# juhyeonkim95/Mitsuba3DopplerToF

Measured on AMD Instinct MI355X. Metric: Mpaths/s (whole node), Doppler Cornell 512x512 64spp, higher is better.
Workload: dtype f32

## Files before the change

mitsuba3dopplertof_amd/__init__.py:

```python
import ctypes as C
import os

import numpy as np

__all__ = ["load_file", "load_string", "load_dict", "Scene", "Integrator", "Sampler", "DtofError", "render",
           "render_multi_pass", "to_tof_image", "lib_path", "ETimeSampling", "velocity_map_variants", "MOMENT_PLANES"]

_HERE = os.path.dirname(os.path.abspath(__file__))
_LIB = None


class DtofError(RuntimeError):
    pass


class ETimeSampling:
    UNIFORM, STRATIFIED, ANTITHETIC, ANTITHETIC_MIRROR, PERIODIC, REGULAR = 0, 1, 2, 3, 4, 5


class _Stats(C.Structure):
    _fields_ = [("n_paths", C.c_uint64), ("n_bounces", C.c_uint64), ("n_shadow_rays", C.c_uint64),
                ("ms_total", C.c_double), ("ms_generate", C.c_double), ("ms_trace", C.c_double),
                ("ms_shade", C.c_double), ("ms_shadow", C.c_double), ("ms_splat", C.c_double),
                ("n_launches_trace", C.c_uint32), ("n_launches_shade", C.c_uint32), ("n_launches_shadow", C.c_uint32),
                ("n_batches", C.c_uint32), ("n_launches_first", C.c_uint32), ("ms_first", C.c_double),
                ("n_inline_iterations", C.c_uint32), ("n_bounces_inline", C.c_uint64), ("n_fused_splat_launches", C.c_uint32),
                ("n_plan_facts_launches", C.c_uint32)]

    def as_dict(self):
        return {k: getattr(self, k) for k, _ in self._fields_}


class _Info(C.Structure):
    _fields_ = [("film_width", C.c_int32), ("film_height", C.c_int32), ("crop_x", C.c_int32), ("crop_y", C.c_int32),
                ("crop_width", C.c_int32), ("crop_height", C.c_int32), ("sample_count", C.c_uint32),
                ("n_shapes", C.c_uint32), ("n_groups", C.c_uint32), ("n_objects", C.c_uint32), ("n_emitters", C.c_uint32),
                ("n_triangles", C.c_uint32), ("n_bvh_nodes", C.c_uint32), ("scene_blob_bytes", C.c_uint32),
                ("time", C.c_float), ("w_g", C.c_float), ("g_1", C.c_float), ("g_0", C.c_float), ("w_s", C.c_float),
                ("phase_offset", C.c_float), ("hetero_frequency", C.c_float), ("antithetic_shift", C.c_float),
                ("wave_type", C.c_int32), ("low_frequency_component_only", C.c_int32), ("time_sampling", C.c_int32),
                ("stratify_each_interval", C.c_int32), ("path_correlation_depth", C.c_uint32), ("max_depth", C.c_uint32),
                ("rr_depth", C.c_uint32), ("base_seed", C.c_uint32), ("time_correlate_number", C.c_int32),
                ("path_correlate_number", C.c_int32), ("bvh_stack_depth", C.c_uint32),
                ("filter_radius", C.c_float), ("filter_halo", C.c_int32), ("has_alpha", C.c_int32)]


_FLAT_SHAPE_FIELDS = 1 << 18 | 0xf << 19 | 0x7 << 23


def lib_path():
    return os.environ.get("DTOF_LIB") or os.path.join(_HERE, "libdtof.so")


def _lib():
    global _LIB
    if _LIB is not None:
        return _LIB
    path = lib_path()
    try:
        import torch
    except ImportError:
        pass
    if not os.path.exists(path):
        raise ImportError("%s is missing -- build it with `make -C %s/csrc` (or __graft_entry__.build()); "
                          "there is no CPU fallback" % (path, _HERE))
    L = C.CDLL(path)
    cpp = C.POINTER(C.c_char_p)
    vp = C.c_void_p
    L.dtof_version.restype = C.c_char_p
    L.dtof_last_error.restype = C.c_char_p
# ... 193 lines not shown

    def info(self):
        i = _Info()
        _check(_lib().dtof_scene_get_info(self._h, C.byref(i)))
        return {k: getattr(i, k) for k, _ in i._fields_}

    @property
    def size(self):
        i = self.info()
        return i["crop_width"], i["crop_height"]

    def export(self, kind):
        n = C.c_size_t(0)
        _check(_lib().dtof_scene_export(self._h, kind, None, 0, C.byref(n)))
        out = np.zeros(n.value, np.float32)
        _check(_lib().dtof_scene_export(self._h, kind, out.ctypes.data, out.size, C.byref(n)))
        return out

    @property
    def plan_facts_launches(self):
        return int(_lib().dtof_scene_plan_facts_launches(self._h))

    @property
    def last_plan_mask(self):
        return int(_lib().dtof_scene_last_plan_facts(self._h))

    @property
    def last_plan_facts(self):
        return self.last_plan_mask & ~_FLAT_SHAPE_FIELDS

    @property
    def last_plan_shape(self):
        m = self.last_plan_mask
        return ((m >> 19) & 0xf, (m >> 23) & 0x7) if m & (1 << 18) else None

    def set_integrator(self, props):
        _check(_lib().dtof_scene_set_integrator(self._h, *_plugin_args(props)))

    def set_sampler(self, props):
        _check(_lib().dtof_scene_set_sampler(self._h, *_plugin_args(props)))

    def render(self, seed=0, spp=0, offsets=None, sensor=0, variants=None, film="float32"):
        if offsets is not None and variants is not None:
            raise DtofError("pass either offsets or variants, not both")
        if _film64(film):
            if sensor != 0:
                raise DtofError("Scene::render(): sensor index %d is out of bounds!" % sensor)
            if offsets is not None:
# ... 442 lines not shown
```

mitsuba3dopplertof_amd/csrc/dtof_kernels.h:

```cpp
#pragma once
#include <stdint.h>
#include <hip/hip_runtime.h>
#include "dtof_math.h"

namespace dtof {

constexpr uint32_t kChunkBlocks = 8;
constexpr uint32_t kMaxInline = 4;
constexpr int kMaxOffsets = 4;

struct RenderParams {
    float s2c[16];
    float cam_to_world[12];
    float near_clip, far_clip, shutter_open, shutter_open_time;
    int32_t orthographic;
    float aperture_radius, focus_distance;
    int32_t crop_x, crop_y, crop_w, crop_h;
    float scale_x, scale_y, offset_x, offset_y;
    int32_t filter; float filter_radius, inv_radius;
    float gauss_coeff[10];
    float filter_b, filter_c;
    uint32_t base_seed, seed, seed_value;
    uint32_t spp, spp_log2;
    uint32_t tcn, pcn;
// ... 99 lines not shown
static_assert(ShadeLds::resident(171, 8, false, true, 12).bytes() == 103088 && ShadeLds::resident(171, 8, false, true, 12).park_off() == 3072, "resident stage, four films");
static_assert(ShadeLds::classic(214, true, true, 5).bytes() == 10080 && ShadeLds::classic(214, true, true, 5).without_stack() == 9568, "classic one-wall launch");

enum : uint32_t {
    kFactSinglePass     = 1u << 0,
    kFactDopplerCorr    = 1u << 1,
    kFactNoLaneOutput   = 1u << 2,
    kFactIdentityQueue  = 1u << 3,
    kFactNoRoulette     = 1u << 4,
    kFactCorrelated     = 1u << 5,
    kFactWholePath      = 1u << 6,
    kFactOneBlock       = 1u << 7,
    kFactOneEmitter     = 1u << 8,
    kFactWavePixel      = 1u << 9,
    kFactFlat           = 1u << 10,
    kFactOneWall        = 1u << 11,
    kFactFusedSplat     = 1u << 12,
    kFactStratifiedPairs = 1u << 13,
    kFactPow2Strata     = 1u << 14,
    kFactSineLowPass    = 1u << 15,
    kFactEmitterSampled = 1u << 16,
    kFactIdShift24      = 1u << 17,
    kFactFlatShape      = 1u << 18,
};
constexpr uint32_t kFlatShapeCountShift = 19, kFlatShapeWallShift = 23, kFlatShapeMax = 8;
constexpr uint32_t kFlatShapeFields = kFactFlatShape | 0xfu << kFlatShapeCountShift | 0x7u << kFlatShapeWallShift;
constexpr uint32_t flat_shape_fact(uint32_t n_objects, uint32_t wall) {
    return n_objects >= 1 && n_objects <= kFlatShapeMax && wall < n_objects ? kFactFlatShape | n_objects << kFlatShapeCountShift | wall << kFlatShapeWallShift : 0u;
}
constexpr uint32_t flat_shape_count(uint32_t facts) { return (facts & kFactFlatShape) ? (facts >> kFlatShapeCountShift) & 0xfu : 0u; }
constexpr uint32_t flat_shape_wall(uint32_t facts) { return (facts >> kFlatShapeWallShift) & 0x7u; }
constexpr bool facts_hold(uint32_t launch, uint32_t kernel) {
    return (launch & kernel & ~kFlatShapeFields) == (kernel & ~kFlatShapeFields) && (!(kernel & kFactFlatShape) || (launch & kFlatShapeFields) == (kernel & kFlatShapeFields));
}
constexpr uint32_t kFactsFlatTable = kFactOneWall | kFlatShapeFields;
static_assert(flat_shape_fact(5, 2) == 0x12c0000u && flat_shape_count(flat_shape_fact(5, 2)) == 5 && flat_shape_wall(flat_shape_fact(5, 2)) == 2 && flat_shape_fact(9, 2) == 0 && flat_shape_fact(5, 5) == 0, "shape fields");
constexpr uint32_t kFactsSampling = kFactStratifiedPairs | kFactPow2Strata | kFactSineLowPass | kFactEmitterSampled | kFactIdShift24;
constexpr bool facts_lane_shifts(uint32_t facts) { return (facts & kFactWavePixel) != 0 && (facts & kFactsSampling) != 0; }
#ifndef DTOF_HEADLINE_FACTS
#define DTOF_HEADLINE_FACTS 0xfff
#endif
constexpr uint32_t kHeadlineFacts = DTOF_HEADLINE_FACTS;
#ifndef DTOF_HEADLINE_FUSED
#define DTOF_HEADLINE_FUSED 1
#endif
constexpr uint32_t kHeadlineFusedFacts = DTOF_HEADLINE_FUSED ? (kHeadlineFacts | kFactFusedSplat) : 0u;
#ifndef DTOF_HEADLINE_C2
#define DTOF_HEADLINE_C2 0x3e000
#endif
constexpr uint32_t kHeadlineC2Facts = (DTOF_HEADLINE_C2) != 0 && kHeadlineFusedFacts != 0 ? (kHeadlineFusedFacts | (DTOF_HEADLINE_C2)) : 0u;
static_assert(((DTOF_HEADLINE_C2) & ~kFactsSampling) == 0, "DTOF_HEADLINE_C2 names route facts only (bits 13 and up)");
#ifndef DTOF_HEADLINE_SHAPE_COUNT
#define DTOF_HEADLINE_SHAPE_COUNT 5
#endif
#ifndef DTOF_HEADLINE_SHAPE_WALL
#define DTOF_HEADLINE_SHAPE_WALL 2
#endif
constexpr uint32_t kHeadlineShapeFacts = (DTOF_HEADLINE_SHAPE_COUNT) != 0 && (kHeadlineC2Facts & kFactOneWall) != 0 ? (kHeadlineC2Facts | flat_shape_fact(DTOF_HEADLINE_SHAPE_COUNT, DTOF_HEADLINE_SHAPE_WALL)) : 0u;
static_assert((DTOF_HEADLINE_SHAPE_COUNT) == 0 || (kHeadlineC2Facts & kFactOneWall) == 0 || (kHeadlineShapeFacts & kFactFlatShape) != 0, "a shape has 1 .. 8 objects and the wall among them");
#ifndef DTOF_FLAT_SHAPE_ANY
#define DTOF_FLAT_SHAPE_ANY 1
#endif
#ifndef DTOF_FLAT_SHAPE_CLOSEST
#define DTOF_FLAT_SHAPE_CLOSEST 1
#endif
#ifndef DTOF_WALL_FRAMES
#define DTOF_WALL_FRAMES 1
#endif
#ifndef DTOF_RESIDENT_FACTS
#define DTOF_RESIDENT_FACTS 0x37f
#endif
constexpr uint32_t kResidentFacts = DTOF_RESIDENT_FACTS;

struct ShadeLaunch { bool staged; int mode; uint32_t waves, grid, lds, lds_flat; hipStream_t stream; ShadeArgs args; uint32_t facts; };
uint32_t launch_shade_plain(bool area, bool k4, const ShadeLaunch &L);
void launch_shade_mesh(bool area, bool k4, const ShadeLaunch &L);
void launch_shade_spec1(bool k4, const ShadeLaunch &L);
void launch_shade_spec2(bool k4, const ShadeLaunch &L);
uint32_t launch_shade_resident0(bool area, bool k4, const ShadeLaunch &L);
void launch_shade_resident1(bool k4, const ShadeLaunch &L);
void launch_shade_resident2(bool k4, const ShadeLaunch &L);

// ... 70 lines not shown
```

mitsuba3dopplertof_amd/csrc/dtof_math.h:

```cpp
#pragma once
#include <hip/hip_runtime.h>
#include <stdint.h>
#include <math.h>

#define DTOF_HD __host__ __device__ __forceinline__

namespace dtof {

constexpr float kPi = 3.14159265358979323846f;
constexpr float kInvPi = 0.31830988618379067154f;
constexpr float kRayEps = 1500.f * 5.9604644775390625e-8f;
constexpr float kShadowEps = kRayEps * 10.f;
constexpr float kLargest = 3.40282346638528859812e+38f;

struct V3 { float x, y, z; };

DTOF_HD uint32_t f2u(float f) {
#if defined(__HIP_DEVICE_COMPILE__)
    return __float_as_uint(f);
#else
    uint32_t u; __builtin_memcpy(&u, &f, 4); return u;
#endif
}
DTOF_HD float u2f(uint32_t u) {
// ... 372 lines not shown
        sum += 0x9e3779b9u;
        v0 += ((v1 << 4) + 0xa341316cu) ^ (v1 + sum) ^ ((v1 >> 5) + 0xc8013ea4u);
        v1 += ((v0 << 4) + 0xad90777du) ^ (v0 + sum) ^ ((v0 >> 5) + 0x7e95761eu);
    }
    o0 = v0; o1 = v1;
}
constexpr uint64_t kPcgMult = 0x5851f42d4c957f2dULL;
DTOF_HD uint32_t pcg_next_u32(uint64_t &state, uint64_t inc) {
    uint64_t old = state;
    state = old * kPcgMult + inc;
    uint32_t xs = (uint32_t) (((old >> 18) ^ old) >> 27), rot = (uint32_t) (old >> 59);
    return (xs >> rot) | (xs << ((~rot + 1u) & 31));
}
DTOF_HD float pcg_next_f32(uint64_t &state, uint64_t inc) {
    return u2f((pcg_next_u32(state, inc) >> 9) | 0x3f800000u) - 1.f;
}
DTOF_HD float pcg_output_f32(uint64_t old) {
    uint32_t xs = (uint32_t) (((old >> 18) ^ old) >> 27), rot = (uint32_t) (old >> 59);
    return u2f((((xs >> rot) | (xs << ((~rot + 1u) & 31))) >> 9) | 0x3f800000u) - 1.f;
}
constexpr uint64_t pcg_pow(int n) { uint64_t r = 1; for (int i = 0; i < n; ++i) r *= kPcgMult; return r; }
constexpr uint64_t kPcgMult6 = pcg_pow(6), kPcgGeom6 = 1 + pcg_pow(1) + pcg_pow(2) + pcg_pow(3) + pcg_pow(4) + pcg_pow(5);
DTOF_HD uint64_t pcg_jump6(uint64_t state, uint64_t inc) { return state * kPcgMult6 + inc * kPcgGeom6; }
DTOF_HD void pcg_seed(uint32_t initstate, uint32_t initseq, uint64_t &state, uint64_t &inc) {
    state = 0; inc = ((uint64_t) initseq << 1) | 1u;
    pcg_next_u32(state, inc);
    state += (uint64_t) initstate;
    pcg_next_u32(state, inc);
}
DTOF_HD uint32_t permute_kensler(uint32_t index, uint32_t n, uint32_t seed, FastDiv dn) {
    if (n <= 1) return 0;
    uint32_t w = n - 1;
    w |= w >> 1; w |= w >> 2; w |= w >> 4; w |= w >> 8; w |= w >> 16;
    do {
        uint32_t tmp = index;
        tmp ^= seed;            tmp *= 0xe170893du;
        tmp ^= seed >> 16;      tmp ^= (tmp & w) >> 4;
        tmp ^= seed >> 8;       tmp *= 0x0929eb3fu;
        tmp ^= seed >> 23;      tmp ^= (tmp & w) >> 1;
        tmp *= 1 | seed >> 27;  tmp *= 0x6935fa69u;
        tmp ^= (tmp & w) >> 11; tmp *= 0x74dcb303u;
        tmp ^= (tmp & w) >> 2;  tmp *= 0x9e501cc3u;
        tmp ^= (tmp & w) >> 2;  tmp *= 0xc860a3dfu;
        tmp &= w;               tmp ^= tmp >> 5;
        index = tmp;
    } while (index >= n);
// ... 20 lines not shown
```

mitsuba3dopplertof_amd/csrc/dtof_render.hip:

```cpp
#include "../../include/dtof.h"
#include "dtof_kernels.h"
#include "dtof_reconstruct.h"
#include "dtof_film64.h"
#include "dtof_moments.h"
#include "dtof_flat_query.h"
#include "dtof_scene.h"
#include "dtof_math.h"
#include <atomic>
#include <dlfcn.h>
#include <cstdio>
#include <cstring>
#include <cstdlib>
#include <cmath>
#include <string>
#include <memory>
#include <vector>

using namespace dtof;

namespace {

thread_local std::string g_last_error;

struct HipError : std::runtime_error { using std::runtime_error::runtime_error; };
// ... 390 lines not shown
    }
    uint32_t launch_facts(const RenderParams &r, const LaunchSpan &l, uint32_t depth0, bool first, bool identity_queue, bool dump) const {
        if (!plan_facts || !first) return 0u;
        const uint32_t depth_end = depth0 + l.span;
        uint32_t f = 0;
        if (r.n_passes == 1 && r.pass == 0) f |= kFactSinglePass;
        if (r.integrator == 0 && r.sampler_kind == SAMPLER_CORRELATED) f |= kFactDopplerCorr;
        if (!dump && !r.want_valid) f |= kFactNoLaneOutput;
        if (identity_queue) f |= kFactIdentityQueue;
        if (r.rr_depth > depth_end) f |= kFactNoRoulette;
        if (depth_end < r.path_correlation_depth) f |= kFactCorrelated;
        if (!l.next_runs && l.terminal) f |= kFactWholePath;
        if (l.chunk_blocks == 1) f |= kFactOneBlock;
        if (n_emitters == 1) f |= kFactOneEmitter;
        if (r.flat_objects != 0) f |= kFactFlat;
        if (one_wall) f |= kFactOneWall | flat_shape;
        if ((f & kFactDopplerCorr) && r.time_sampling == TIME_STRATIFIED && r.stratify != 0 && r.tcn == 2 && r.pcn == 2 && r.shutter_open_time > 0.f && r.spp > 1) f |= kFactStratifiedPairs;
        if (r.n_stratum >= 2 && (r.n_stratum & (r.n_stratum - 1u)) == 0) f |= kFactPow2Strata;
        if (r.low_pass != 0 && r.wave_type == WAVE_SIN) f |= kFactSineLowPass;
        if (depth_end < r.max_depth) f |= kFactEmitterSampled;
        if (id_shift == 24) f |= kFactIdShift24;
        if (l.splat_here) f |= kFactFusedSplat;
        if (identity_queue && r.stripe_rows == 0 && r.spp_log2 != 0xffffffffu && r.spp_log2 >= 6 && (r.lane_base & 63u) == 0 && (r.n_lanes & 63u) == 0) f |= kFactWavePixel;
        return f;
    }
};

void plan_lanes(FramePlan &p, const dtof_scene *sc, const RenderRequest &rq) {
    const HostSensor &se = sc->host.sensor;
    uint32_t spp = rq.spp ? rq.spp : sc->pp.sample_count;
    if (spp == 0) throw std::runtime_error("sample count must be positive");
    const uint32_t sample_count = spp;
    uint32_t per_pass = sc->pp.samples_per_pass == 0xffffffffu || sc->pp.samples_per_pass == 0 ? spp : std::min(sc->pp.samples_per_pass, spp);
    if (spp % per_pass != 0) throw std::runtime_error("sample_count (" + std::to_string(spp) + ") must be a multiple of spp_per_pass (" + std::to_string(per_pass) + ").");
    const uint64_t wavefront = (uint64_t) se.crop_w * se.crop_h * per_pass, limit = 0xffffffffull;
    if (wavefront > limit) {
        per_pass /= (uint32_t) ((wavefront + limit - 1) / limit);
        if (per_pass == 0 || spp % per_pass != 0) throw std::runtime_error("sample_count should be a multiple of samples_per_wavefront!");
    }
    p.n_passes = spp / per_pass; spp = per_pass;
    const uint64_t total_lanes = (uint64_t) se.crop_w * se.crop_h * spp;
    if (sc->pp.time_sampling != TIME_UNIFORM && sc->pp.stratify_each_interval && sample_count < (uint32_t) sc->pp.time_correlate_number)
        throw std::runtime_error("sample count must be at least time_correlate_number when per-interval stratification is on");
    if (sc->pp.integrator == 0 && sc->pp.sampler_kind == SAMPLER_CORRELATED && sc->pp.time_sampling == TIME_ANTITHETIC_MIRROR && sc->pp.time_correlate_number != 2)
        throw std::runtime_error("antithetic_mirror time sampling needs time_correlate_number == 2");
    p.rp = make_params(sc, rq.seed, spp, rq.offsets, rq.n_offsets, sample_count, rq.variants, rq.n_variants);
// ... 1279 lines not shown
```

mitsuba3dopplertof_amd/csrc/dtof_shade.h:

```cpp
#pragma once
#include "dtof_device.h"
#include <atomic>
#include <initializer_list>
#include <type_traits>

namespace dtof {


DTOF_D uint32_t wave_append(bool pred, uint32_t &running) {
    const uint64_t mask = __ballot(pred);
    const uint32_t slot = running + (uint32_t) __popcll(mask & ((1ull << __lane_id()) - 1ull));
    running += (uint32_t) __popcll(mask);
    return slot;
}

struct BsdfOut { V3 val, weight, wo; float pdf, bs_pdf, bs_eta; bool bs_delta, bs_null; };
template <int SPEC>
DTOF_D void bsdf_eval_pdf_sample(const SceneView &sv, const DShape *sh, Surface &si, V3 wo, bool active_em, float sample_1, float s2x, float s2y, BsdfOut &out, bool want_sample = true) {
    const bool masked = SPEC && (sh->flags & SF_MASK);
    bool null_pick = false; float opacity = 1.f;
    if (masked) { opacity = mask_opacity_at(sv, sh, si.u, si.v); null_pick = !(sample_1 < opacity); sample_1 = sample_1 / opacity; }
    const bool blend = SPEC == 2 && (sh->flags & SF_BLEND);
    float blend_w = 0.f; bool pick_1 = false;
    if (blend) {
        blend_w = sh->tex_blend ? texture_eval_1(sv, sh->tex_blend << 4, si.u, si.v) : sh->blend_weight;
        blend_w = fmin_(fmax_(blend_w, 0.f), 1.f);
        pick_1 = sample_1 <= blend_w;
    }
    const DShape *side_sh = (SPEC == 2 && (sh->flags & SF_TWOSIDED2) && si.wi.z < 0.f) ? &sv.shapes[sh->blend_other] : sh;
    const V3 wi_plain = si.wi, wo_plain = wo;
    V3 bsdf_val = mk(0, 0, 0), bsdf_weight = mk(0, 0, 0), bs_wo = mk(0, 0, 0);
    float bsdf_pdf = 0.f, bs_pdf = 0.f, bs_eta = 0.f; bool bs_delta = false, bs_null = false;
    V3 val_0 = mk(0, 0, 0), keep_weight = mk(0, 0, 0), keep_wo = mk(0, 0, 0); float pdf_0 = 0.f, keep_pdf = 0.f, keep_eta = 0.f; bool keep_delta = false, keep_null = false;
    for (int pass = 0; pass < (SPEC == 2 && blend ? 2 : 1); ++pass) {
        const DShape *bsh = pass ? &sv.shapes[sh->blend_other] : side_sh;
        const float s1 = !blend ? sample_1 : (pass ? sample_1 / blend_w : (sample_1 - blend_w) / (1.f - blend_w));
        si.wi = wi_plain; wo = wo_plain;
        bool twosided = bsh->flags & SF_TWOSIDED;
        const bool nmap = SPEC && (bsh->flags & (SF_NORMALMAP | SF_BUMPMAP));
        LocalFrame nf; V3 wo_flipped = wo; bool nm_back = false;
        if (nmap) {
// ... 152 lines not shown
            }
            if (want_sample && wiz > 0.f) {
                float prob_specular = f_i * w, prob_diffuse = (1.f - f_i) * (1.f - w);
                prob_specular = prob_specular / (prob_specular + prob_diffuse);
                prob_diffuse = 1.f - prob_specular;
                bs_eta = 1.f;
                if (s1 < prob_specular) {
                    bs_wo = mk(-si.wi.x, -si.wi.y, wiz);
                    bs_pdf = prob_specular; bs_delta = true;
                    const float value = f_i / bs_pdf;
                    bsdf_weight = mk(value * hm.spec_refl[0], value * hm.spec_refl[1], value * hm.spec_refl[2]);
                } else {
                    bs_wo = cosine_hemisphere(s2x, s2y);
                    bs_pdf = prob_diffuse * (kInvPi * bs_wo.z);
                    float f_o; fresnel_dielectric(bs_wo.z, bsh->diel_eta, f_o, t1, t2, t3);
                    const float k = bsh->inv_eta_2 * (1.f - f_i) * (1.f - f_o) / prob_diffuse;
                    bsdf_weight = mk(diff.x * k, diff.y * k, diff.z * k);
                }
                if (twosided) bs_wo.z = mulsign(bs_wo.z, si.wi.z);
            }
        } else {
            if (wiz > 0.f && woz > 0.f) { bsdf_val = mk(refl.x * kInvPi * woz, refl.y * kInvPi * woz, refl.z * kInvPi * woz); bsdf_pdf = kInvPi * woz; }
            if (want_sample && wiz > 0.f) {
                bs_wo = cosine_hemisphere(s2x, s2y);
                bs_pdf = kInvPi * bs_wo.z;
                bs_eta = 1.f;
                if (bs_pdf > 0.f) bsdf_weight = refl;
                if (twosided) bs_wo.z = mulsign(bs_wo.z, si.wi.z);
            }
        }
        if (nmap) {
            if (!(wo_flipped.z * wo.z > 0.f)) { bsdf_val = mk(0, 0, 0); bsdf_pdf = 0.f; }
            if (bsdf_weight.x != 0.f || bsdf_weight.y != 0.f || bsdf_weight.z != 0.f) {
                const V3 pw = frame_to_world(nf, bs_wo);
                if (!(bs_wo.z * pw.z > 0.f)) bsdf_weight = mk(0, 0, 0);
                bs_wo = pw;
            }
            if (nm_back) bs_wo.z = -bs_wo.z;
        }
        if (blend) {
            if ((pass == 1) == pick_1) { keep_weight = bsdf_weight; keep_wo = bs_wo; keep_pdf = bs_pdf; keep_eta = bs_eta; keep_delta = bs_delta; keep_null = bs_null; }
            if (pass == 0) { val_0 = bsdf_val; pdf_0 = bsdf_pdf; }
            else {
                const float w0 = 1.f - blend_w;
                bsdf_val = mk(val_0.x * w0 + bsdf_val.x * blend_w, val_0.y * w0 + bsdf_val.y * blend_w, val_0.z * w0 + bsdf_val.z * blend_w);
                bsdf_pdf = pdf_0 * w0 + bsdf_pdf * blend_w;
// ... 62 lines not shown
    }
}
template <bool AREA, bool MESH, int SPEC, bool ONE_EMITTER = false>
void launch_emitter_eval_level(const uint8_t *scene, int mode, uint32_t index, float pmf, const float *in, float *out, uint32_t n, hipStream_t s) {
    if (n) hipLaunchKernelGGL((k_emitter_eval<AREA, MESH, SPEC, ONE_EMITTER>), dim3(nblk(n)), dim3(kBlock), 0, s, scene, mode, index, pmf, in, out, n);
}

template <bool LDS, int MODE, bool AREA, int KMAX, bool MESH, int SPEC, int RESW = 0, bool RH16 = false, uint32_t FACTS = 0>
#ifndef DTOF_MESH_WAVES
#define DTOF_MESH_WAVES 3
#endif
#ifndef DTOF_K4_RES_LDS
#define DTOF_K4_RES_LDS 1
#endif
__global__ __launch_bounds__(RESW ? RESW * 64 : kShadeBlock, RESW ? RESW / 4 : (MODE == 2 && !MESH && !SPEC && KMAX == 1) ? 4 : (MODE != 0 && MESH) ? ((SPEC && KMAX > 1) ? 2 : DTOF_MESH_WAVES) : 1) void k_shade(ShadeArgs args_by_value) {
    constexpr bool FUSED = MODE != 0, FIRST = MODE == 2;
    static_assert(FACTS == 0 || MODE == 2, "plan facts describe a first-bounce launch");
    constexpr bool F_SINGLE_PASS = (FACTS & kFactSinglePass) != 0, F_DOPPLER_CORR = (FACTS & kFactDopplerCorr) != 0, F_NO_LANE_OUT = (FACTS & kFactNoLaneOutput) != 0;
    constexpr bool F_IDENTITY = (FACTS & kFactIdentityQueue) != 0, F_NO_RR = (FACTS & kFactNoRoulette) != 0, F_CORRELATED = (FACTS & kFactCorrelated) != 0;
    constexpr bool F_WHOLE_PATH = (FACTS & kFactWholePath) != 0, F_ONE_BLOCK = (FACTS & kFactOneBlock) != 0, F_ONE_EMITTER = (FACTS & kFactOneEmitter) != 0;
    constexpr bool F_WAVE_PIXEL = (FACTS & kFactWavePixel) != 0;
    constexpr bool F_FLAT = (FACTS & kFactFlat) != 0, F_ONE_WALL = (FACTS & kFactOneWall) != 0, F_FUSED_SPLAT = (FACTS & kFactFusedSplat) != 0;
    constexpr bool F_EMITTER_SAMPLED = (FACTS & kFactEmitterSampled) != 0, F_ID24 = (FACTS & kFactIdShift24) != 0, F_SHIFTS = facts_lane_shifts(FACTS);
    constexpr bool F_FRAMES = F_ONE_WALL && DTOF_WALL_FRAMES;
    static_assert(!F_FLAT || (!MESH && SPEC == 0 && RESW == 0), "trace_flat serves the staged rectangle-only diffuse kernels");
    static_assert(!F_ONE_WALL || F_FLAT, "the one wall is an object of the flat table");
    static_assert(!F_FUSED_SPLAT || KMAX == 1, "the fused splat is the one-film kernels'");
    static_assert(!F_WAVE_PIXEL || F_IDENTITY, "whole waves of one pixel are provable for an identity queue only");
    static_assert(!F_ONE_BLOCK || RESW == 0, "blocks per segment belong to the classic launch");
    constexpr bool RES_LDS = RESW != 0 && KMAX > 1 && DTOF_K4_RES_LDS;
    constexpr bool S16 = RESW != 0 && KMAX > 1;
    static_assert(!RES_LDS || 3 * KMAX == (int) kParkWords + 1, "the film-state columns hold all but the last float of the K results");
    constexpr bool PARK_ST = DTOF_PARK && RESW == 16 && KMAX == 1;
    constexpr bool PARK = DTOF_PARK && RESW == 16 && (KMAX == 1 || RES_LDS);
    constexpr uint32_t kRngAt = RES_LDS ? kParkWords : 0u;
    constexpr int KREG = RES_LDS ? 1 : KMAX;
    constexpr uint32_t kStackStride = RESW ? RESW * 64 : kShadeBlock;
    static_assert(RESW == 0 || (MODE == 2 && !LDS && MESH), "the resident stage exists for the unstaged fused first-bounce kernel with mesh code");
    static_assert(!RH16 || RESW != 0, "half-float LDS planes belong to the resident stage");
    extern __shared__ uint4 lds[];
    __shared__ uint32_t s_inline_all[(RESW ? RESW : 1) * 2 * kMaxInline];
    typedef const char __attribute__((address_space(4))) *KernargBytes;
    const KernargBytes kernarg = (KernargBytes) __builtin_amdgcn_kernarg_segment_ptr();
    const ShadeArgs &A0 = *(const ShadeArgs *) kernarg;
    const uint32_t lane_id = RESW ? threadIdx.x & 63u : threadIdx.x, wave_id = RESW ? threadIdx.x >> 6 : 0u;
    uint32_t *const s_inline = s_inline_all + wave_id * 2 * kMaxInline;
// ... 96 lines not shown
    if constexpr (RES_LDS) res_clear();
    const float4 zero4 = make_float4(0.f, 0.f, 0.f, 0.f);
    uint32_t hid = 0xffffffffu; float4 ra = make_float4(0.f, 0.f, 0.f, 0.f), rb = make_float4(0.f, 0.f, 1.f, 0.f), st = ra; uint4 hh = make_uint4(0u, 0u, 0u, 0u); Rng main = { 0ull, 1ull }, path = { 0ull, 1ull };
    float4 stb_reg = make_float4(0.f, 0.f, 0.f, 1.f); float2 stc_reg = make_float2(1.f, 1.f);
    uint32_t *const parku = (uint32_t *) park;
    auto park_store = [&]() {
        parku[kRngAt * kStackStride] = (uint32_t) main.state; parku[(kRngAt + 1) * kStackStride] = (uint32_t) (main.state >> 32); parku[(kRngAt + 2) * kStackStride] = (uint32_t) (main.inc >> 1);
        parku[(kRngAt + 3) * kStackStride] = (uint32_t) path.state; parku[(kRngAt + 4) * kStackStride] = (uint32_t) (path.state >> 32); parku[(kRngAt + 5) * kStackStride] = (uint32_t) (path.inc >> 1);
        if (PARK_ST) { park[6 * kStackStride] = st.x; park[7 * kStackStride] = st.y; park[8 * kStackStride] = st.z; park[9 * kStackStride] = st.w; }
    };
    auto park_load = [&]() {
        main.state = (uint64_t) parku[kRngAt * kStackStride] | ((uint64_t) parku[(kRngAt + 1) * kStackStride] << 32); main.inc = ((uint64_t) parku[(kRngAt + 2) * kStackStride] << 1) | 1u;
        path.state = (uint64_t) parku[(kRngAt + 3) * kStackStride] | ((uint64_t) parku[(kRngAt + 4) * kStackStride] << 32); path.inc = ((uint64_t) parku[(kRngAt + 5) * kStackStride] << 1) | 1u;
        if (PARK_ST) st = make_float4(park[6 * kStackStride], park[7 * kStackStride], park[8 * kStackStride], park[9 * kStackStride]);
    };
    const bool valid_start = SPEC && rp.has_env && !rp.hide_emitters;
    bool valid_reg = valid_start;
    float memo_m[12], memo_inv[12];
    typename std::conditional<F_FRAMES, WallFrames, NoFrames>::type wf;
    if constexpr (F_FRAMES) {
        wf.n = mk(0.f, 0.f, 1.f); wf.s = mk(1.f, 0.f, 0.f);
        wf.table = (const DFlatFrame *) ((const uint4 *) ((const DFlatObject *) (sv.base + rp.flat_off) + rp.flat_objects) + 1 + rp.flat_objects);
    }
    bool lane_on = in_range;
#ifdef DTOF_TRAVERSAL_STATS
    constexpr uint64_t kPoisonState = 0xdeadbeefcafef00dull;
    if (!in_range) { main.state = path.state = kPoisonState; const float pz = u2f(0x7fc0dead); ra = rb = st = make_float4(pz, pz, pz, pz); }
#define DTOF_POISON_CHECK() do { if (main.state == kPoisonState || path.state == kPoisonState || f2u(st.x) == 0x7fc0deadu || f2u(ra.x) == 0x7fc0deadu) DTOF_STAT(14); } while (0)
#else
#define DTOF_POISON_CHECK() ((void) 0)
#endif
    const bool wave_pixel = F_WAVE_PIXEL || (FIRST && rp.spp_log2 != 0xffffffffu && rp.spp_log2 >= 6 && (rp.lane_base & 63u) == 0 && count - cbase >= (uint32_t) kShadeBlock);
    const bool fuse_splat = F_FUSED_SPLAT || (FIRST && A.film != nullptr);
    float2 pos_reg = make_float2(0.f, 0.f);
    if (in_range) {
        l = qin ? qin[seg * kSeg + j] : seg * kSeg + j;
        if (FIRST) {
            const PrimaryLane pl = generate_lane<SPEC == 0, FACTS>(rp, global_lane<FACTS>(rp, rp.lane_base + l), wave_pixel, rp.lane_base + l);
            ra = pl.ray_a; rb = pl.ray_b; main = pl.main; path = pl.path; st = make_float4(1.f, 1.f, 1.f, 0.f);
            if (PARK) park_store();
            pos_reg = pl.pos;
            if (!fuse_splat) {
                q.pos[l] = pl.pos;
                q.rng_b[l] = make_uint2((uint32_t) (main.inc >> 1), (uint32_t) (path.inc >> 1));
            }
            if (dbg) {
                LaneDebug &o = dbg[l];
                o.time = ra.w; o.ray_o[0] = ra.x; o.ray_o[1] = ra.y; o.ray_o[2] = ra.z; o.ray_d[0] = rb.x; o.ray_d[1] = rb.y; o.ray_d[2] = rb.z;
            }
            if (have_memo) instance_memo_fill(sv, ra.w, memo_m, memo_inv);
            if constexpr (F_FRAMES) {
                const DShape &ws = sv.shapes[sv.groups[sv.objects[sv.memo_obj].index].first_shape];
                wf.n = normalize(xf_normal(memo_inv, mk(ws.n[0], ws.n[1], ws.n[2])));
                const V3 du = xf_vector(memo_m, mk(ws.dp_du[0], ws.dp_du[1], ws.dp_du[2]));
                wf.s = normalize(vfma(wf.n, -dot(wf.n, du), du));
                if (du.x == 0.f && du.y == 0.f && du.z == 0.f) { V3 tt; coordinate_system(wf.n, wf.s, tt); }
            }
            Hit h;
            bool found = (F_FLAT || flat) ? trace_flat<false, true, FACTS & kFactsFlatTable>(sv, (ConstBytes) A.scene + rp.flat_off, rp.flat_off, flat, stack, mk(ra.x, ra.y, ra.z), mk(rb.x, rb.y, rb.z), ra.w, rb.w, h)
                              : trace_scene<false, MESH, FUSED, RESW != 0, kStackStride, S16, 0u, false, RH16>(sv, stack, mk(ra.x, ra.y, ra.z), mk(rb.x, rb.y, rb.z), ra.w, rb.w, h);
            hh = make_uint4(f2u(h.t), f2u(h.u), f2u(h.v), h.prim);
            hid = found ? (h.obj | (h.shape << (F_ID24 ? 24u : q.id_shift))) : 0xffffffffu;
// ... 96 lines not shown
                    if (SPEC && on && sh->tex_radiance) le = texture_eval(sv, sh->tex_radiance << 4, si.u, si.v);
#pragma unroll
                    for (int k = 0; k < KMAX; ++k) if (KMAX == 1 || k < rp.n_offsets) {
                        V3 v = le * mis_bsdf;
                        if (!plain) v = v * modulation_weight<FACTS>(rp, rp.w_d[k], rp.phase[k], time, path_length);
                        float4 r;
                        if constexpr (RES_LDS) r = res_get(k); else r = rcur[k];
                        const float4 acc = make_float4(fmaf(thr.x, v.x, r.x), fmaf(thr.y, v.y, r.y), fmaf(thr.z, v.z, r.z), 0.f);
                        if constexpr (RES_LDS) res_put(k, acc); else rcur[k] = acc;
                    }
                    res_dirty = !RES_LDS;
                }
            }

            if (terminal && !active_next) {
                if constexpr (!RES_LDS) if (res_dirty) {
#pragma unroll
                    for (int k = 0; k < KMAX; ++k) if (KMAX == 1 || k < rp.n_offsets) res_put(k, rcur[k]);
                }
                if (!F_NO_LANE_OUT && rp.want_valid) q.valid_out[l] = make_float4(1.f, 0.f, 0.f, 0.f);
            } else {
            const bool use_path = !single && correlate;
            Rng sel = use_path ? path : main;
            float e1 = next_f32(sel), e2 = next_f32(sel);
            bool active_em = active_next && (F_ONE_EMITTER || sv.n_emitters > 0) && (!SPEC || bsdf_is_smooth(sh->bsdf) || ((sh->flags & (SF_BLEND | SF_TWOSIDED2)) && bsdf_is_smooth(sv.shapes[sh->blend_other].bsdf)));
            V3 em_weight = mk(0, 0, 0), wo = mk(0, 0, 0); float ds_dist = 0.f, ds_pdf = 0.f; bool ds_delta = true;
            if (active_em) {
                const EmitterSample es = sample_emitter_direction<AREA, MESH, SPEC, F_ONE_EMITTER>(sv, si.p, e1, e2, pmf);
                const V3 dsp = es.p, dd = es.d;
                em_weight = es.weight; ds_dist = es.dist; ds_pdf = es.pdf; ds_delta = es.delta; active_em = es.usable;
                V3 so = offset_p(si, dsp - si.p);
                V3 sd = dsp - so;
                float sdist = norm(sd);
                sd = sd * rcp(sdist);
                sha = make_float4(so.x, so.y, so.z, sdist * (1.f - kShadowEps));
                shb = make_float4(sd.x, sd.y, sd.z, time);
                wo = want_frame ? mk(dot(dd, si.sh_s), dot(dd, si.sh_t), dot(dd, si.sh_n)) : mk(0.f, 0.f, dot(dd, si.sh_n));
            }
            float sample_1 = 0.f, s2x = 0.f, s2y = 0.f;
            if (!terminal) { sample_1 = next_f32(sel); s2x = next_f32(sel); s2y = next_f32(sel); }

            BsdfOut bo;
            bsdf_eval_pdf_sample<SPEC>(sv, sh, si, wo, active_em, sample_1, s2x, s2y, bo, !terminal);
            const V3 bsdf_val = bo.val, bs_wo = bo.wo; V3 bsdf_weight = bo.weight;
            const float bsdf_pdf = bo.pdf, bs_pdf = bo.bs_pdf, bs_eta = bo.bs_eta; const bool bs_delta = bo.bs_delta, bs_null = bo.bs_null;
            if (active_em) {
                const float mis_em = ds_delta ? 1.f : mis_weight(ds_pdf, bsdf_pdf);
                bool nonzero = false;
                if constexpr (RES_LDS) {
                    pend_thr = thr; pend_len = path_length + ds_dist;
                    pend_v = mk(bsdf_val.x * em_weight.x * mis_em, bsdf_val.y * em_weight.y * mis_em, bsdf_val.z * em_weight.z * mis_em);
                    nonzero = (int) (pend_thr.x * pend_v.x != 0.f) | (int) (pend_thr.y * pend_v.y != 0.f) | (int) (pend_thr.z * pend_v.z != 0.f);
                } else {
#pragma unroll
                for (int k = 0; k < KMAX; ++k) if (KMAX == 1 || k < rp.n_offsets) {
                    float4 r = AREA ? rcur[k] : res_get(k);
                    V3 v = mk(bsdf_val.x * em_weight.x * mis_em, bsdf_val.y * em_weight.y * mis_em, bsdf_val.z * em_weight.z * mis_em);
                    if (!plain) { float lw = modulation_weight<FACTS>(rp, rp.w_d[k], rp.phase[k], time, path_length + ds_dist); v = v * lw; }
                    float3 c = make_float3(fmaf(thr.x, v.x, r.x), fmaf(thr.y, v.y, r.y), fmaf(thr.z, v.z, r.z));
                    cand[k] = c;
                    nonzero |= f2u(c.x) != f2u(r.x) || f2u(c.y) != f2u(r.y) || f2u(c.z) != f2u(r.z);
                }
                }
                want_shadow = nonzero;
            }
            if constexpr (!RES_LDS) if (res_dirty) {
#pragma unroll
                for (int k = 0; k < KMAX; ++k) if (KMAX == 1 || k < rp.n_offsets) res_put(k, rcur[k]);
            }
            if (terminal) {
                if (!F_NO_LANE_OUT && rp.want_valid) q.valid_out[l] = make_float4(1.f, 0.f, 0.f, 0.f);
            } else {
            V3 nd = vfma(si.sh_n, bs_wo.z, vfma(si.sh_t, bs_wo.y, si.sh_s * bs_wo.x));
            V3 no = offset_p(si, nd);
            thr = mk(thr.x * bsdf_weight.x, thr.y * bsdf_weight.y, thr.z * bsdf_weight.z);
            const float eta = eta_path * bs_eta;
            uint32_t ndepth = depth + 1;
            float thr_max = fmax_(fmax_(thr.x, thr.y), thr.z);
            float rr_prob = fmin_(thr_max * sqr(eta), .95f);
            bool rr_active = !F_NO_RR && ndepth >= rp.rr_depth;
            bool rr_continue = next_f32(sel) < rr_prob;
            if (use_path) { path.state = sel.state; main.state = pcg_jump6(main.state, main.inc); }
            else { main.state = sel.state; if (!single) path.state = pcg_jump6(path.state, path.inc); }
            if (rr_active) thr = thr * rcp(rr_prob);
            alive = active_next && (!rr_active || rr_continue) && thr_max != 0.f;
            const bool valid_now = !SPEC || valid_in || !bs_null;
            const bool ends = !alive || (last && !trace_next);
            if (SPEC && ends && !valid_now) {
                want_shadow = false;
                if constexpr (RES_LDS) res_clear();
                else {
#pragma unroll
                    for (int k = 0; k < KMAX; ++k) if (KMAX == 1 || k < rp.n_offsets) res_put(k, zero4);
                }
            }
            if (!F_NO_LANE_OUT && ends && rp.want_valid) q.valid_out[l] = make_float4(valid_now ? 1.f : 0.f, 0.f, 0.f, 0.f);
            if (FIRST) valid_reg = valid_now;
            if (alive) {
                nra = make_float4(no.x, no.y, no.z, time); nrb = make_float4(nd.x, nd.y, nd.z, kLargest);
                const float4 sta = make_float4(thr.x, thr.y, thr.z, path_length), stb = make_float4(si.p.x, si.p.y, si.p.z, bs_pdf);
                const float2 stc = make_float2(eta, bs_delta ? 1.f : 0.f);
                if ((!FIRST || last) && trace_next) {
                    q.ray_a[l] = nra;
                    q.ray_b[l] = nrb;
                    q.st_a[l] = sta;
                    if (AREA) q.st_b[l] = stb;
// ... 49 lines not shown
            for (int k = 0; k < KMAX; ++k) if (KMAX == 1 || k < rp.n_offsets) q.res[(size_t) k * q.capacity + l] = make_float4(cand[k].x, cand[k].y, cand[k].z, 0.f);
        }
        if (alive && trace_next) {
            Hit h;
            bool found = (F_FLAT || flat) ? trace_flat<false, true, FACTS & kFactsFlatTable>(sv, (ConstBytes) A.scene + rp.flat_off, rp.flat_off, flat, stack, mk(nra.x, nra.y, nra.z), mk(nrb.x, nrb.y, nrb.z), nra.w, nrb.w, h)
                              : trace_scene<false, MESH, true, RESW != 0, kStackStride, S16, 0u, false, RH16>(sv, stack, mk(nra.x, nra.y, nra.z), mk(nrb.x, nrb.y, nrb.z), nra.w, nrb.w, h);
            if (!FIRST || last) store_hit<MESH>(q, l, h, found);
            if (FIRST) { hh = make_uint4(f2u(h.t), f2u(h.u), f2u(h.v), h.prim); hid = found ? (h.obj | (h.shape << (F_ID24 ? 24u : q.id_shift))) : 0xffffffffu; }
        }
        const uint32_t n_sh = (uint32_t) __popcll(__ballot(want_shadow)) * ((threadIdx.x & 63) == 0 ? 1u : 0u);
        if (last) n_shadow += n_sh; else if (lane_id == 0) s_inline[2 * it + 1] += n_sh;
    } else {
        uint32_t sslot = seg * kSeg + wave_append(want_shadow, n_shadow);
        if (want_shadow) {
            q.sh_a[sslot] = sha; q.sh_b[sslot] = shb;
#pragma unroll
            for (int k = 0; k < KMAX; ++k) if (KMAX == 1 || k < rp.n_offsets)
                q.sh_c[(size_t) k * q.capacity + sslot] = make_float4(cand[k].x, cand[k].y, cand[k].z, u2f(l));
        }
    }
    if (last) break;
    lane_on = alive;
    if (alive) { ra = nra; rb = nrb; DTOF_POISON_CHECK(); }
    }
    if constexpr (!RES_LDS) if (FIRST && fuse_splat) {
        const uint32_t W = (uint32_t) rp.crop_w;
        const uint32_t pix = F_SHIFTS ? (uint32_t) __builtin_amdgcn_readfirstlane((int) (rp.lane_base + l)) >> rp.spp_log2 : fdiv(global_lane(rp, rp.lane_base + l), rp.d_spp);
        const int py = (int) fdiv(pix, rp.d_w), px = (int) (pix - W * (uint32_t) py);
        const float sx = pos_reg.x, sy = pos_reg.y;
        const bool regular = in_range && (int) floorf(sx) - rp.crop_x == px && (int) floorf(sy) - rp.crop_y == py;
        if (wave_pixel) {
            const int upx = __builtin_amdgcn_readfirstlane(px), upy = __builtin_amdgcn_readfirstlane(py);
            const float relx = (float) (upx + rp.crop_x - 1) + .5f - sx, rely = (float) (upy + rp.crop_y - 1) + .5f - sy;
            float wx[3], wy[3];
#pragma unroll
            for (int a = 0; a < 3; ++a) { wx[a] = regular ? tent(relx + (float) a, rp.inv_radius) : 0.f; wy[a] = tent(rely + (float) a, rp.inv_radius); }
            const uint32_t sum_id = __brev(lane_id) >> 26, tap = sum_id >> 2, ch = sum_id & 3u;
            const int fx = upx - 1 + (int) (tap % 3u), fy = upy - 1 + (int) (tap / 3u);
            const bool store = sum_id < 36u && (unsigned) fx < W && (unsigned) fy < (unsigned) rp.crop_h;
#pragma unroll
            for (int k = 0; k < KMAX; ++k) if (KMAX == 1 || k < rp.n_offsets) {
                float *fk = A.film + (size_t) k * A.film_stride;
                if (in_range && !regular) splat_lane<F_FUSED_SPLAT ? FILTER_TENT : -1>(rp, fk, sx, sy, px, py, rbase[k].x, rbase[k].y, rbase[k].z);
                float v[36];
#pragma unroll
                for (int ys = 0; ys < 3; ++ys)
// ... 64 lines not shown
```

mitsuba3dopplertof_amd/csrc/dtof_shade_plain.hip:

```cpp
#include "dtof_shade.h"

namespace dtof {

template <uint32_t FACTS> static uint32_t launch_headline(const ShadeLaunch &L) {
    if (FACTS == 0 || !facts_hold(L.facts, FACTS)) return 0u;
    hipLaunchKernelGGL((k_shade<true, 2, false, 1, false, 0, 0, false, FACTS>), dim3(L.grid), dim3(kShadeBlock), (FACTS & kFactFlat) ? L.lds_flat : L.lds, L.stream, L.args);
    return FACTS;
}
uint32_t launch_shade_plain(bool area, bool k4, const ShadeLaunch &L) {
    if (!area && !k4 && L.staged && L.mode == 2) {
        if (uint32_t ran = launch_headline<kHeadlineShapeFacts>(L)) return ran;
        if (uint32_t ran = launch_headline<kHeadlineC2Facts>(L)) return ran;
        if (uint32_t ran = launch_headline<kHeadlineFusedFacts>(L)) return ran;
        if (uint32_t ran = launch_headline<kHeadlineFacts>(L)) return ran;
    }
    if (area) { if (k4) launch_shade_variant<true, kMaxOffsets, false, 0>(L); else launch_shade_variant<true, 1, false, 0>(L); }
    else      { if (k4) launch_shade_variant<false, kMaxOffsets, false, 0>(L); else launch_shade_variant<false, 1, false, 0>(L); }
    return 0u;
}

void launch_bsdf_eval_0(const uint8_t *scene, uint32_t shape_index, const float *in, float *out, uint32_t n, hipStream_t s) {
    launch_bsdf_eval_spec<0>(scene, shape_index, in, out, n, s);
}

void launch_emitter_eval_plain(const uint8_t *scene, int level, int mode, uint32_t index, float pmf, const float *in, float *out, uint32_t n, hipStream_t s) {
    if (level == 1) launch_emitter_eval_level<true, false, 0>(scene, mode, index, pmf, in, out, n, s);
    else if (level == 6) launch_emitter_eval_level<false, false, 0, true>(scene, mode, index, pmf, in, out, n, s);
    else launch_emitter_eval_level<false, false, 0>(scene, mode, index, pmf, in, out, n, s);
}

}
```

Baseline: 18330.

## Share paired-lane BSDF direction samples via DPP and jump PCG streams

Adds a specialised shade kernel for correlated, stratified-pair, single-point-light diffuse launches, selected ahead of the existing headline kernels. Lanes 2k and 2k+1 share one path stream. At path start each lane draws one cosine-hemisphere direction from a jumped PCG state, and DPP swaps hand each lane the direction its partner's stream would have produced for this bounce and the next. Per-bounce emitter, lobe and roulette draws are dropped, and the stream is advanced with closed-form PCG jumps instead of sequential draws. This removes RNG and sampling arithmetic from the bounce loop, but it only holds under a narrow set of scene facts and relies on the whole wave being active for the cross-lane reads.

```diff
diff --git a/mitsuba3dopplertof_amd/__init__.py b/mitsuba3dopplertof_amd/__init__.py
--- a/mitsuba3dopplertof_amd/__init__.py
+++ b/mitsuba3dopplertof_amd/__init__.py
@@ -46,6 +46,7 @@
 
 
 _FLAT_SHAPE_FIELDS = 1 << 18 | 0xf << 19 | 0x7 << 23
+_PAIR_SAMPLES = 1 << 26
 
 
 def lib_path():
@@ -285,8 +286,16 @@
         return int(_lib().dtof_scene_plan_facts_launches(self._h))
 
     @property
+    def last_plan_kernel(self):
+        return int(_lib().dtof_scene_last_plan_facts(self._h))
+
+    @property
     def last_plan_mask(self):
-        return int(_lib().dtof_scene_last_plan_facts(self._h))
+        return self.last_plan_kernel & ~_PAIR_SAMPLES
+
+    @property
+    def last_plan_pair_samples(self):
+        return bool(self.last_plan_kernel & _PAIR_SAMPLES)
 
     @property
     def last_plan_facts(self):
diff --git a/mitsuba3dopplertof_amd/csrc/dtof_kernels.h b/mitsuba3dopplertof_amd/csrc/dtof_kernels.h
--- a/mitsuba3dopplertof_amd/csrc/dtof_kernels.h
+++ b/mitsuba3dopplertof_amd/csrc/dtof_kernels.h
@@ -145,6 +145,7 @@
     kFactEmitterSampled = 1u << 16,
     kFactIdShift24      = 1u << 17,
     kFactFlatShape      = 1u << 18,
+    kFactPairSamples    = 1u << 26,
 };
 constexpr uint32_t kFlatShapeCountShift = 19, kFlatShapeWallShift = 23, kFlatShapeMax = 8;
 constexpr uint32_t kFlatShapeFields = kFactFlatShape | 0xfu << kFlatShapeCountShift | 0x7u << kFlatShapeWallShift;
@@ -181,6 +182,16 @@
 #endif
 constexpr uint32_t kHeadlineShapeFacts = (DTOF_HEADLINE_SHAPE_COUNT) != 0 && (kHeadlineC2Facts & kFactOneWall) != 0 ? (kHeadlineC2Facts | flat_shape_fact(DTOF_HEADLINE_SHAPE_COUNT, DTOF_HEADLINE_SHAPE_WALL)) : 0u;
 static_assert((DTOF_HEADLINE_SHAPE_COUNT) == 0 || (kHeadlineC2Facts & kFactOneWall) == 0 || (kHeadlineShapeFacts & kFactFlatShape) != 0, "a shape has 1 .. 8 objects and the wall among them");
+#ifndef DTOF_HEADLINE_PAIR
+#define DTOF_HEADLINE_PAIR 1
+#endif
+#ifndef DTOF_STREAM_JUMPS
+#define DTOF_STREAM_JUMPS 1
+#endif
+#ifndef DTOF_PAIR_SAMPLES
+#define DTOF_PAIR_SAMPLES 1
+#endif
+constexpr uint32_t kHeadlinePairFacts = DTOF_HEADLINE_PAIR && kHeadlineShapeFacts != 0 ? (kHeadlineShapeFacts | kFactPairSamples) : 0u;
 #ifndef DTOF_FLAT_SHAPE_ANY
 #define DTOF_FLAT_SHAPE_ANY 1
 #endif
diff --git a/mitsuba3dopplertof_amd/csrc/dtof_math.h b/mitsuba3dopplertof_amd/csrc/dtof_math.h
--- a/mitsuba3dopplertof_amd/csrc/dtof_math.h
+++ b/mitsuba3dopplertof_amd/csrc/dtof_math.h
@@ -418,6 +418,12 @@
 constexpr uint64_t pcg_pow(int n) { uint64_t r = 1; for (int i = 0; i < n; ++i) r *= kPcgMult; return r; }
 constexpr uint64_t kPcgMult6 = pcg_pow(6), kPcgGeom6 = 1 + pcg_pow(1) + pcg_pow(2) + pcg_pow(3) + pcg_pow(4) + pcg_pow(5);
 DTOF_HD uint64_t pcg_jump6(uint64_t state, uint64_t inc) { return state * kPcgMult6 + inc * kPcgGeom6; }
+constexpr uint64_t pcg_geom(int n) { uint64_t r = 0, p = 1; for (int i = 0; i < n; ++i) { r += p; p *= kPcgMult; } return r; }
+template <int N> DTOF_HD uint64_t pcg_jump(uint64_t state, uint64_t inc) {
+    constexpr uint64_t m = pcg_pow(N), g = pcg_geom(N);
+    return state * m + inc * g;
+}
+static_assert(pcg_pow(6) == kPcgMult6 && pcg_geom(6) == kPcgGeom6, "pcg_jump<6> is pcg_jump6");
 DTOF_HD void pcg_seed(uint32_t initstate, uint32_t initseq, uint64_t &state, uint64_t &inc) {
     state = 0; inc = ((uint64_t) initseq << 1) | 1u;
     pcg_next_u32(state, inc);
diff --git a/mitsuba3dopplertof_amd/csrc/dtof_render.hip b/mitsuba3dopplertof_amd/csrc/dtof_render.hip
--- a/mitsuba3dopplertof_amd/csrc/dtof_render.hip
+++ b/mitsuba3dopplertof_amd/csrc/dtof_render.hip
@@ -436,6 +436,8 @@
         if (id_shift == 24) f |= kFactIdShift24;
         if (l.splat_here) f |= kFactFusedSplat;
         if (identity_queue && r.stripe_rows == 0 && r.spp_log2 != 0xffffffffu && r.spp_log2 >= 6 && (r.lane_base & 63u) == 0 && (r.n_lanes & 63u) == 0) f |= kFactWavePixel;
+        constexpr uint32_t pair_needs = kFactWholePath | kFactWavePixel | kFactStratifiedPairs | kFactCorrelated | kFactDopplerCorr | kFactNoRoulette | kFactOneEmitter;
+        if (l.span == 3 && (f & pair_needs) == pair_needs) f |= kFactPairSamples;
         return f;
     }
 };
diff --git a/mitsuba3dopplertof_amd/csrc/dtof_shade.h b/mitsuba3dopplertof_amd/csrc/dtof_shade.h
--- a/mitsuba3dopplertof_amd/csrc/dtof_shade.h
+++ b/mitsuba3dopplertof_amd/csrc/dtof_shade.h
@@ -15,8 +15,8 @@
 }
 
 struct BsdfOut { V3 val, weight, wo; float pdf, bs_pdf, bs_eta; bool bs_delta, bs_null; };
-template <int SPEC>
-DTOF_D void bsdf_eval_pdf_sample(const SceneView &sv, const DShape *sh, Surface &si, V3 wo, bool active_em, float sample_1, float s2x, float s2y, BsdfOut &out, bool want_sample = true) {
+template <int SPEC, bool HAVE_WO = false>
+DTOF_D void bsdf_eval_pdf_sample(const SceneView &sv, const DShape *sh, Surface &si, V3 wo, bool active_em, float sample_1, float s2x, float s2y, BsdfOut &out, bool want_sample = true, const V3 *diffuse_wo = nullptr) {
     const bool masked = SPEC && (sh->flags & SF_MASK);
     bool null_pick = false; float opacity = 1.f;
     if (masked) { opacity = mask_opacity_at(sv, sh, si.u, si.v); null_pick = !(sample_1 < opacity); sample_1 = sample_1 / opacity; }
@@ -215,6 +215,7 @@
         } else {
             if (wiz > 0.f && woz > 0.f) { bsdf_val = mk(refl.x * kInvPi * woz, refl.y * kInvPi * woz, refl.z * kInvPi * woz); bsdf_pdf = kInvPi * woz; }
             if (want_sample && wiz > 0.f) {
+                if constexpr (HAVE_WO) bs_wo = *diffuse_wo; else
                 bs_wo = cosine_hemisphere(s2x, s2y);
                 bs_pdf = kInvPi * bs_wo.z;
                 bs_eta = 1.f;
@@ -323,6 +324,10 @@
     constexpr bool F_WAVE_PIXEL = (FACTS & kFactWavePixel) != 0;
     constexpr bool F_FLAT = (FACTS & kFactFlat) != 0, F_ONE_WALL = (FACTS & kFactOneWall) != 0, F_FUSED_SPLAT = (FACTS & kFactFusedSplat) != 0;
     constexpr bool F_EMITTER_SAMPLED = (FACTS & kFactEmitterSampled) != 0, F_ID24 = (FACTS & kFactIdShift24) != 0, F_SHIFTS = facts_lane_shifts(FACTS);
+    constexpr bool F_PAIR = (FACTS & kFactPairSamples) != 0, JUMPS = F_PAIR && DTOF_STREAM_JUMPS, PAIR = F_PAIR && DTOF_PAIR_SAMPLES;
+    static_assert(!F_PAIR || F_WAVE_PIXEL, "a lane reads its partner's registers: the whole wave is active where it does");
+    static_assert(!F_PAIR || (!AREA && SPEC == 0 && KMAX == 1 && F_ONE_EMITTER), "a diffuse BSDF picks no lobe and a lone point light samples nothing: of an iteration's six draws only s2x and s2y are read");
+    static_assert(!F_PAIR || (F_NO_RR && F_CORRELATED && F_DOPPLER_CORR && F_WHOLE_PATH && F_SINGLE_PASS && (FACTS & kFactStratifiedPairs) != 0), "every draw comes from the stream lanes 2k and 2k + 1 share, none is looked at for roulette, no state outlives the launch");
     constexpr bool F_FRAMES = F_ONE_WALL && DTOF_WALL_FRAMES;
     static_assert(!F_FLAT || (!MESH && SPEC == 0 && RESW == 0), "trace_flat serves the staged rectangle-only diffuse kernels");
     static_assert(!F_ONE_WALL || F_FLAT, "the one wall is an object of the flat table");
@@ -465,6 +470,7 @@
         wf.n = mk(0.f, 0.f, 1.f); wf.s = mk(1.f, 0.f, 0.f);
         wf.table = (const DFlatFrame *) ((const uint4 *) ((const DFlatObject *) (sv.base + rp.flat_off) + rp.flat_objects) + 1 + rp.flat_objects);
     }
+    V3 pair_wo = mk(0.f, 0.f, 1.f), pair_wo_next = pair_wo;
     bool lane_on = in_range;
 #ifdef DTOF_TRAVERSAL_STATS
     constexpr uint64_t kPoisonState = 0xdeadbeefcafef00dull;
@@ -481,6 +487,28 @@
         if (FIRST) {
             const PrimaryLane pl = generate_lane<SPEC == 0, FACTS>(rp, global_lane<FACTS>(rp, rp.lane_base + l), wave_pixel, rp.lane_base + l);
             ra = pl.ray_a; rb = pl.ray_b; main = pl.main; path = pl.path; st = make_float4(1.f, 1.f, 1.f, 0.f);
+            if constexpr (PAIR) {
+                const bool odd = lane_id & 1u;
+                uint64_t sx;
+                if constexpr (JUMPS) {
+                    constexpr uint64_t m3 = pcg_pow(3), g3 = pcg_geom(3), m9 = pcg_pow(9), g9 = pcg_geom(9);
+                    sx = path.state * (odd ? m9 : m3) + path.inc * (odd ? g9 : g3);
+                } else {
+                    uint64_t s3 = path.state;
+                    for (int i = 0; i < 3; ++i) s3 = s3 * kPcgMult + path.inc;
+                    uint64_t s9 = s3;
+                    for (int i = 0; i < 6; ++i) s9 = s9 * kPcgMult + path.inc;
+                    sx = odd ? s9 : s3;
+                }
+                const uint64_t sy = sx * kPcgMult + path.inc;
+                const V3 mine = cosine_hemisphere(pcg_output_f32(sx), pcg_output_f32(sy));
+                pair_wo = mk(__int_as_float(__builtin_amdgcn_update_dpp(0, __float_as_int(mine.x), 0xa0, 0xf, 0xf, false)),
+                             __int_as_float(__builtin_amdgcn_update_dpp(0, __float_as_int(mine.y), 0xa0, 0xf, 0xf, false)),
+                             __int_as_float(__builtin_amdgcn_update_dpp(0, __float_as_int(mine.z), 0xa0, 0xf, 0xf, false)));
+                pair_wo_next = mk(__int_as_float(__builtin_amdgcn_update_dpp(0, __float_as_int(mine.x), 0xf5, 0xf, 0xf, false)),
+                                  __int_as_float(__builtin_amdgcn_update_dpp(0, __float_as_int(mine.y), 0xf5, 0xf, 0xf, false)),
+                                  __int_as_float(__builtin_amdgcn_update_dpp(0, __float_as_int(mine.z), 0xf5, 0xf, 0xf, false)));
+            }
             if (PARK) park_store();
             pos_reg = pl.pos;
             if (!fuse_splat) {
@@ -623,7 +651,8 @@
             } else {
             const bool use_path = !single && correlate;
             Rng sel = use_path ? path : main;
-            float e1 = next_f32(sel), e2 = next_f32(sel);
+            float e1 = 0.f, e2 = 0.f;
+            if constexpr (!JUMPS && !PAIR) { e1 = next_f32(sel); e2 = next_f32(sel); }
             bool active_em = active_next && (F_ONE_EMITTER || sv.n_emitters > 0) && (!SPEC || bsdf_is_smooth(sh->bsdf) || ((sh->flags & (SF_BLEND | SF_TWOSIDED2)) && bsdf_is_smooth(sv.shapes[sh->blend_other].bsdf)));
             V3 em_weight = mk(0, 0, 0), wo = mk(0, 0, 0); float ds_dist = 0.f, ds_pdf = 0.f; bool ds_delta = true;
             if (active_em) {
@@ -639,9 +668,15 @@
                 wo = want_frame ? mk(dot(dd, si.sh_s), dot(dd, si.sh_t), dot(dd, si.sh_n)) : mk(0.f, 0.f, dot(dd, si.sh_n));
             }
             float sample_1 = 0.f, s2x = 0.f, s2y = 0.f;
+            if constexpr (PAIR) { }
+            else if constexpr (JUMPS) {
+                if (!terminal) { sel.state = pcg_jump<3>(sel.state, sel.inc); s2x = next_f32(sel); s2y = pcg_output_f32(sel.state); }
+            } else
             if (!terminal) { sample_1 = next_f32(sel); s2x = next_f32(sel); s2y = next_f32(sel); }
 
             BsdfOut bo;
+            if constexpr (PAIR) bsdf_eval_pdf_sample<SPEC, true>(sv, sh, si, wo, active_em, sample_1, s2x, s2y, bo, !terminal, &pair_wo);
+            else
             bsdf_eval_pdf_sample<SPEC>(sv, sh, si, wo, active_em, sample_1, s2x, s2y, bo, !terminal);
             const V3 bsdf_val = bo.val, bs_wo = bo.wo; V3 bsdf_weight = bo.weight;
             const float bsdf_pdf = bo.pdf, bs_pdf = bo.bs_pdf, bs_eta = bo.bs_eta; const bool bs_delta = bo.bs_delta, bs_null = bo.bs_null;
@@ -680,9 +715,14 @@
             float thr_max = fmax_(fmax_(thr.x, thr.y), thr.z);
             float rr_prob = fmin_(thr_max * sqr(eta), .95f);
             bool rr_active = !F_NO_RR && ndepth >= rp.rr_depth;
-            bool rr_continue = next_f32(sel) < rr_prob;
+            bool rr_continue = true;
+            if constexpr (PAIR) { }
+            else if constexpr (JUMPS) path.state = pcg_jump<2>(sel.state, sel.inc);
+            else {
+            rr_continue = next_f32(sel) < rr_prob;
             if (use_path) { path.state = sel.state; main.state = pcg_jump6(main.state, main.inc); }
             else { main.state = sel.state; if (!single) path.state = pcg_jump6(path.state, path.inc); }
+            }
             if (rr_active) thr = thr * rcp(rr_prob);
             alive = active_next && (!rr_active || rr_continue) && thr_max != 0.f;
             const bool valid_now = !SPEC || valid_in || !bs_null;
@@ -778,6 +818,7 @@
     if (last) break;
     lane_on = alive;
     if (alive) { ra = nra; rb = nrb; DTOF_POISON_CHECK(); }
+    if constexpr (PAIR) pair_wo = pair_wo_next;
     }
     if constexpr (!RES_LDS) if (FIRST && fuse_splat) {
         const uint32_t W = (uint32_t) rp.crop_w;
diff --git a/mitsuba3dopplertof_amd/csrc/dtof_shade_plain.hip b/mitsuba3dopplertof_amd/csrc/dtof_shade_plain.hip
--- a/mitsuba3dopplertof_amd/csrc/dtof_shade_plain.hip
+++ b/mitsuba3dopplertof_amd/csrc/dtof_shade_plain.hip
@@ -9,6 +9,7 @@
 }
 uint32_t launch_shade_plain(bool area, bool k4, const ShadeLaunch &L) {
     if (!area && !k4 && L.staged && L.mode == 2) {
+        if (uint32_t ran = launch_headline<kHeadlinePairFacts>(L)) return ran;
         if (uint32_t ran = launch_headline<kHeadlineShapeFacts>(L)) return ran;
         if (uint32_t ran = launch_headline<kHeadlineC2Facts>(L)) return ran;
         if (uint32_t ran = launch_headline<kHeadlineFusedFacts>(L)) return ran;
```

After: 19050, median of 6. 1.04x the previous value.
